# YannDubs/disentangling-vae

Hardware: NVIDIA H100
Metric: images/sec (higher is better)
Workload: dtype f32

## Files before the change

disentangling-vae_b200/csrc/dv_conv_img.cu:

```cuda
#include "dv_common.cuh"

namespace dv {
namespace img {

constexpr int kThreads = 256;
constexpr int kLoPitch = 36;

__device__ __forceinline__ void cp_async16(void* smem_dst, const void* gsrc, bool valid) {
  const uint32_t d = (uint32_t)__cvta_generic_to_shared(smem_dst);
  const int sz = valid ? 16 : 0;
  asm volatile("cp.async.cg.shared.global [%0], [%1], 16, %2;" ::"r"(d), "l"(gsrc), "r"(sz) : "memory");
}
__device__ __forceinline__ void cp_async4(void* smem_dst, const void* gsrc, bool valid) {
  const uint32_t d = (uint32_t)__cvta_generic_to_shared(smem_dst);
  const int sz = valid ? 4 : 0;
  asm volatile("cp.async.ca.shared.global [%0], [%1], 4, %2;" ::"r"(d), "l"(gsrc), "r"(sz) : "memory");
}
__device__ __forceinline__ void cp_async_wait_all() { asm volatile("cp.async.wait_all;" ::: "memory"); }

template <int CH, int W, int TR>
__device__ __forceinline__ void load_hi_tile(float* __restrict__ s_hi, const float* __restrict__ hi, int b, int i0, int H) {
  constexpr int IN_ROWS = 2 * TR + 2, COLS = 2 * W + 2, PITCH = 2 * W + 4;
  const int HH = 2 * H, WW = 2 * W;
#pragma unroll 4
  for (int e = threadIdx.x; e < CH * IN_ROWS * COLS; e += kThreads) {
    const int xx = e % COLS, rr = (e / COLS) % IN_ROWS, c = e / (COLS * IN_ROWS);
    const int iy = 2 * i0 - 1 + rr, ix = xx - 1;
    const bool ok = (unsigned)iy < (unsigned)HH && (unsigned)ix < (unsigned)WW;
    cp_async4(s_hi + (c * IN_ROWS + rr) * PITCH + xx, ok ? hi + ((long long)(b * CH + c) * HH + iy) * WW + ix : hi, ok);
  }
}

template <int CH, int W>
__global__ void __launch_bounds__(kThreads, 2)
img_down_kernel(const float* __restrict__ hi, const float* __restrict__ wd, const float* __restrict__ bias,
                const float* __restrict__ mask, float* __restrict__ lo, int B, int H, int act,
                float* __restrict__ colsum_part, const uint32_t* __restrict__ mask_bits, uint32_t* __restrict__ bits_out) {
  constexpr int TR = 16;
  constexpr int PXG = (TR * W) / 64;
  constexpr int CB = W / PXG;
  constexpr int NX = 2 * PXG + 2;
  constexpr int IN_ROWS = 2 * TR + 2, PITCH = 2 * W + 4;
  __shared__ __align__(16) float s_w[kTaps * CH * kLoCh];
  __shared__ __align__(16) float s_hi[CH * IN_ROWS * PITCH];
  __shared__ __align__(16) float s_bias[kLoCh];
  __shared__ float s_cs[kThreads / 32][kLoCh];
  const int tid = threadIdx.x, lane = tid & 31, warp = tid >> 5;
  for (int i = tid; i < kTaps * CH * kLoCh; i += kThreads) s_w[i] = wd[i];
  if (tid < kLoCh) s_bias[tid] = bias ? bias[tid] : 0.f;
  const int cg = tid & 3, pg = tid >> 2;
  const int r_thr = pg / CB, c0 = (pg % CB) * PXG;
  const int tiles_per_img = H / TR;
  const int num_tiles = B * tiles_per_img;
  float csum[8];
#pragma unroll
  for (int k = 0; k < 8; ++k) csum[k] = 0.f;
  for (int tile = blockIdx.x; tile < num_tiles; tile += gridDim.x) {
    const int b = tile / tiles_per_img, i0 = (tile % tiles_per_img) * TR;
    __syncthreads();
    load_hi_tile<CH, W, TR>(s_hi, hi, b, i0, H);
    const long long p0 = ((long long)b * H + i0 + r_thr) * W + c0;
    uint32_t mb_lo = 0xffffffffu, mb_hi = 0xffffffffu;
    if (mask_bits) {
      mb_lo = 0u; mb_hi = 0u;
#pragma unroll
      for (int i = 0; i < PXG; ++i) {
        const uint32_t mw = __ldg(mask_bits + p0 + i);
        mb_lo |= ((mw >> (4 * cg)) & 15u) << (4 * i);
        mb_hi |= ((mw >> (16 + 4 * cg)) & 15u) << (4 * i);
      }
    } else if (mask) {
      mb_lo = 0u; mb_hi = 0u;
#pragma unroll
      for (int i = 0; i < PXG; ++i) {
        const float* mk = mask + (p0 + i) * kLoCh + 4 * cg;
        const float4 a = ldg4(mk), d = ldg4(mk + 16);
        mb_lo |= ((a.x > 0.f ? 1u : 0u) | (a.y > 0.f ? 2u : 0u) | (a.z > 0.f ? 4u : 0u) | (a.w > 0.f ? 8u : 0u)) << (4 * i);
        mb_hi |= ((d.x > 0.f ? 1u : 0u) | (d.y > 0.f ? 2u : 0u) | (d.z > 0.f ? 4u : 0u) | (d.w > 0.f ? 8u : 0u)) << (4 * i);
      }
    }
    cp_async_wait_all();
    __syncthreads();
    float acc[PXG][8];
#pragma unroll
    for (int i = 0; i < PXG; ++i)
#pragma unroll
      for (int k = 0; k < 8; ++k) acc[i][k] = 0.f;
#pragma unroll
    for (int c = 0; c < CH; ++c) {
#pragma unroll
      for (int kh = 0; kh < 4; ++kh) {
        float x[NX];
        const float* row = s_hi + (c * IN_ROWS + 2 * r_thr + kh) * PITCH + 2 * c0;
#pragma unroll
        for (int v = 0; v < NX / 2; ++v) {
          const float2 t2 = *reinterpret_cast<const float2*>(row + 2 * v);
          x[2 * v] = t2.x; x[2 * v + 1] = t2.y;
        }
#pragma unroll
        for (int kw = 0; kw < 4; ++kw) {
          const float* wp = s_w + ((kh * 4 + kw) * CH + c) * kLoCh + 4 * cg;
          const float4 wa = *reinterpret_cast<const float4*>(wp), wb = *reinterpret_cast<const float4*>(wp + 16);
#pragma unroll
          for (int i = 0; i < PXG; ++i) {
            const float xv = x[2 * i + kw];
            acc[i][0] = fmaf(xv, wa.x, acc[i][0]); acc[i][1] = fmaf(xv, wa.y, acc[i][1]);
            acc[i][2] = fmaf(xv, wa.z, acc[i][2]); acc[i][3] = fmaf(xv, wa.w, acc[i][3]);
            acc[i][4] = fmaf(xv, wb.x, acc[i][4]); acc[i][5] = fmaf(xv, wb.y, acc[i][5]);
            acc[i][6] = fmaf(xv, wb.z, acc[i][6]); acc[i][7] = fmaf(xv, wb.w, acc[i][7]);
          }
        }
      }
    }
    const float4 ba = *reinterpret_cast<const float4*>(s_bias + 4 * cg), bb = *reinterpret_cast<const float4*>(s_bias + 16 + 4 * cg);
    const float bv[8] = {ba.x, ba.y, ba.z, ba.w, bb.x, bb.y, bb.z, bb.w};
#pragma unroll
    for (int i = 0; i < PXG; ++i) {
      float v[8];
#pragma unroll
      for (int k = 0; k < 8; ++k) {
        float t = acc[i][k] + bv[k];
        if (act == DV_ACT_RELU) t = fmaxf(t, 0.f);
        const uint32_t bit = ((k < 4 ? mb_lo : mb_hi) >> (4 * i + (k & 3))) & 1u;
        v[k] = bit ? t : 0.f;
        csum[k] += v[k];
      }
      float* dst = lo + (p0 + i) * kLoCh + 4 * cg;
      *reinterpret_cast<float4*>(dst) = make_float4(v[0], v[1], v[2], v[3]);
      *reinterpret_cast<float4*>(dst + 16) = make_float4(v[4], v[5], v[6], v[7]);
      if (bits_out) {
        uint32_t ob = 0u;
#pragma unroll
        for (int k = 0; k < 8; ++k) ob |= (v[k] > 0.f ? 1u : 0u) << ((k < 4 ? 0 : 16) + 4 * cg + (k & 3));
        ob |= __shfl_xor_sync(0xffffffffu, ob, 1);
        ob |= __shfl_xor_sync(0xffffffffu, ob, 2);
        if (cg == 0) bits_out[p0 + i] = ob;
      }
    }
  }
  if (colsum_part) {
#pragma unroll
    for (int k = 0; k < 8; ++k) {
      float t = csum[k];
      t += __shfl_xor_sync(0xffffffffu, t, 4); t += __shfl_xor_sync(0xffffffffu, t, 8); t += __shfl_xor_sync(0xffffffffu, t, 16);
      if (lane < 4) s_cs[warp][(k < 4 ? 0 : 16) + 4 * lane + (k & 3)] = t;
    }
    __syncthreads();
    if (warp == 0) {
      float t = 0.f;
#pragma unroll
      for (int w2 = 0; w2 < kThreads / 32; ++w2) t += s_cs[w2][lane];
      colsum_part[blockIdx.x * kLoCh + lane] = t;
    }
  }
}

template <int CH, int W>
__global__ void __launch_bounds__(kThreads, (CH == 1) ? 2 : 1)
img_wgrad_kernel(const float* __restrict__ lo, const float* __restrict__ hi, float* __restrict__ ws, int B, int H) {
  constexpr int TR = (W == 32) ? 16 : 16;
  constexpr int IN_ROWS = 2 * TR + 2, PITCH = 2 * W + 4;
  constexpr int NPX = TR * W;
  constexpr int NSTREAM = kThreads / 16;
  extern __shared__ __align__(16) float smem[];
  float* s_lo = smem;
  float* s_hi = smem + NPX * kLoPitch;
  const int tid = threadIdx.x;
  const int stream = tid >> 4, st = tid & 15;
  const int cl4 = st & 7, half = st >> 3;
  float acc[CH][8][4];
  float bsum[4] = {0.f, 0.f, 0.f, 0.f};
#pragma unroll
  for (int c = 0; c < CH; ++c)
#pragma unroll
    for (int t = 0; t < 8; ++t)
#pragma unroll
      for (int e = 0; e < 4; ++e) acc[c][t][e] = 0.f;
  const int tiles_per_img = H / TR;
  const int num_tiles = B * tiles_per_img;
  for (int tile = blockIdx.x; tile < num_tiles; tile += gridDim.x) {
    const int b = tile / tiles_per_img, i0 = (tile % tiles_per_img) * TR;
    __syncthreads();
    load_hi_tile<CH, W, TR>(s_hi, hi, b, i0, H);
    {
      const float4* src = reinterpret_cast<const float4*>(lo + ((long long)b * H + i0) * W * kLoCh);
#pragma unroll 4
      for (int e = tid; e < NPX * 8; e += kThreads) {
        const int px = e >> 3, j = e & 7;
        cp_async16(s_lo + px * kLoPitch + 4 * j, src + e, true);
      }
    }
    cp_async_wait_all();
    __syncthreads();
#pragma unroll 2
    for (int px = stream; px < NPX; px += NSTREAM) {
      const int r = px / W, cc = px % W;
      const float4 l4 = *reinterpret_cast<const float4*>(s_lo + px * kLoPitch + 4 * cl4);
      if (half == 0) { bsum[0] += l4.x; bsum[1] += l4.y; bsum[2] += l4.z; bsum[3] += l4.w; }
#pragma unroll
      for (int c = 0; c < CH; ++c) {
#pragma unroll
        for (int rr = 0; rr < 2; ++rr) {
          const float* row = s_hi + (c * IN_ROWS + 2 * r + 2 * half + rr) * PITCH + 2 * cc;
          const float2 a = *reinterpret_cast<const float2*>(row), d = *reinterpret_cast<const float2*>(row + 2);
          const float xv[4] = {a.x, a.y, d.x, d.y};
#pragma unroll
          for (int kw = 0; kw < 4; ++kw) {
            acc[c][rr * 4 + kw][0] = fmaf(xv[kw], l4.x, acc[c][rr * 4 + kw][0]);
            acc[c][rr * 4 + kw][1] = fmaf(xv[kw], l4.y, acc[c][rr * 4 + kw][1]);
            acc[c][rr * 4 + kw][2] = fmaf(xv[kw], l4.z, acc[c][rr * 4 + kw][2]);
            acc[c][rr * 4 + kw][3] = fmaf(xv[kw], l4.w, acc[c][rr * 4 + kw][3]);
          }
        }
      }
    }
  }
  __syncthreads();
  constexpr int K = kTaps * CH;
  float* red = smem;
  {
    float* mine = red + stream * (K + 1) * kLoCh;
#pragma unroll
    for (int c = 0; c < CH; ++c)
#pragma unroll
      for (int t = 0; t < 8; ++t) {
        const int tap = (2 * half + (t >> 2)) * 4 + (t & 3);
#pragma unroll
        for (int e = 0; e < 4; ++e) mine[(tap * CH + c) * kLoCh + 4 * cl4 + e] = acc[c][t][e];
      }
    if (half == 0) {
#pragma unroll
      for (int e = 0; e < 4; ++e) mine[K * kLoCh + 4 * cl4 + e] = bsum[e];
    }
  }
  __syncthreads();
  float* out = ws + (long long)blockIdx.x * (K + 1) * kLoCh;
  for (int idx = tid; idx < (K + 1) * kLoCh; idx += kThreads) {
    float s = 0.f;
#pragma unroll
    for (int q = 0; q < NSTREAM; ++q) s += red[q * (K + 1) * kLoCh + idx];
    out[idx] = s;
  }
}

template <int CH, int W>
__global__ void __launch_bounds__(128, 2)
img_up_kernel(const float* __restrict__ lo, const float* __restrict__ wu, const float* __restrict__ bias,
              float* __restrict__ hi, int B, int H, int act) {
  constexpr int NT = 128;
  constexpr int PY = 2;
  constexpr int TCOLS = W / 2;
  constexpr int TROWS = NT / TCOLS;
  constexpr int TR = TROWS * PY;
  constexpr int SW = W + 2;
  extern __shared__ __align__(16) float smem[];
  float* s_lo = smem;
  float* s_w = smem + (TR + 2) * SW * kLoCh;
  const int tid = threadIdx.x;
  for (int i = tid; i < kTaps * CH * kLoCh; i += NT) s_w[i] = wu[i];
  const int tn = tid % TCOLS, tm = tid / TCOLS;
  const int tiles_per_img = (H + TR - 1) / TR;
  const int num_tiles = B * tiles_per_img;
  const int HH = 2 * H, WW = 2 * W;
  for (int tile = blockIdx.x; tile < num_tiles; tile += gridDim.x) {
    const int b = tile / tiles_per_img, m0 = (tile % tiles_per_img) * TR;
    __syncthreads();
#pragma unroll 4
    for (int e = tid; e < (TR + 2) * SW * 8; e += NT) {
      const int j = e & 7, xx = (e >> 3) % SW, rr = (e >> 3) / SW;
      const int m = m0 - 1 + rr, n = xx - 1;
      const bool ok = (unsigned)m < (unsigned)H && (unsigned)n < (unsigned)W;
      cp_async16(s_lo + (rr * SW + xx) * kLoCh + 4 * (j ^ ((xx >> 1) & 7)),
                 ok ? lo + (((long long)b * H + m) * W + n) * kLoCh + 4 * j : lo, ok);
    }
    cp_async_wait_all();
    __syncthreads();
    if (m0 + PY * tm < H) {
      float out[CH][2 * PY][4];
#pragma unroll
      for (int c = 0; c < CH; ++c)
#pragma unroll
        for (int y = 0; y < 2 * PY; ++y)
#pragma unroll
          for (int x = 0; x < 4; ++x) out[c][y][x] = 0.f;
      const float* base = s_lo + ((PY * tm) * SW + 2 * tn) * kLoCh;
#pragma unroll 1
      for (int j = 0; j < 8; ++j) {
        float4 nb[PY + 2][4];
#pragma unroll
        for (int rr = 0; rr < PY + 2; ++rr)
#pragma unroll
          for (int xx = 0; xx < 4; ++xx)
            nb[rr][xx] = *reinterpret_cast<const float4*>(base + (rr * SW + xx) * kLoCh + 4 * (j ^ ((tn + (xx >> 1)) & 7)));
#pragma unroll
        for (int c = 0; c < CH; ++c) {
#pragma unroll
          for (int tap = 0; tap < kTaps; ++tap) {
            const int kh = tap >> 2, kw = tap & 3;
            const float4 w4 = *reinterpret_cast<const float4*>(s_w + (tap * CH + c) * kLoCh + 4 * j);
            const int py = (kh & 1) ? 0 : 1, dm = (kh == 1 || kh == 2) ? 0 : ((kh == 3) ? -1 : 1);
            const int px = (kw & 1) ? 0 : 1, dn = (kw == 1 || kw == 2) ? 0 : ((kw == 3) ? -1 : 1);
#pragma unroll
            for (int a = 0; a < PY; ++a)
#pragma unroll
              for (int d = 0; d < 2; ++d) {
                const float4 v = nb[a + 1 + dm][d + 1 + dn];
                float o = out[c][2 * a + py][2 * d + px];
                o = fmaf(v.x, w4.x, o); o = fmaf(v.y, w4.y, o); o = fmaf(v.z, w4.z, o); o = fmaf(v.w, w4.w, o);
                out[c][2 * a + py][2 * d + px] = o;
              }
          }
        }
      }
#pragma unroll
      for (int c = 0; c < CH; ++c) {
        const float bv = bias ? __ldg(bias + c) : 0.f;
#pragma unroll
        for (int y = 0; y < 2 * PY; ++y) {
          const int oy = 2 * (m0 + PY * tm) + y;
          if (oy < HH) {
            float v[4];
#pragma unroll
            for (int x = 0; x < 4; ++x) v[x] = apply_act(out[c][y][x] + bv, act, 0.f);
            *reinterpret_cast<float4*>(hi + ((long long)(b * CH + c) * HH + oy) * WW + 4 * tn) = make_float4(v[0], v[1], v[2], v[3]);
          }
        }
      }
    }
  }
}

template <int W> constexpr int up_tile_rows() { return (128 / (W / 2)) * 2; }
template <int CH, int W> constexpr size_t up_smem() {
  return (size_t)((up_tile_rows<W>() + 2) * (W + 2) * kLoCh + kTaps * CH * kLoCh) * sizeof(float);
}
template <int CH, int W> constexpr size_t wgrad_smem() {
  constexpr size_t tiles = (size_t)16 * W * kLoPitch + (size_t)CH * 34 * (2 * W + 4);
  constexpr size_t red = (size_t)(kThreads / 16) * (kTaps * CH + 1) * kLoCh;
  return (tiles > red ? tiles : red) * sizeof(float);
}

template <typename K>
static bool set_smem(K kernel, size_t bytes) {
  return bytes <= 48 * 1024 || cudaFuncSetAttribute(kernel, cudaFuncAttributeMaxDynamicSharedMemorySize, (int)bytes) == cudaSuccess;
}

int conv_down(const float* hi, const float* wd, const float* bias, const float* mask, const uint32_t* mask_bits, float* lo,
              uint32_t* bits_out, int B, int H, int W, int CH,
              int act, cudaStream_t st, float* colsum_part, int* nparts, int max_parts) {
  const int tiles = B * (H / 16);
  int grid = tiles < 2 * kNumSMs ? tiles : 2 * kNumSMs;
  if (colsum_part && grid > max_parts) grid = max_parts;
#define DV_IMG_DOWN(CHV, WV) \
  img_down_kernel<CHV, WV><<<grid, kThreads, 0, st>>>(hi, wd, bias, mask, lo, B, H, act, colsum_part, mask_bits, bits_out)
  if (CH == 1 && W == 32) DV_IMG_DOWN(1, 32);
  else if (CH == 3 && W == 32) DV_IMG_DOWN(3, 32);
  else if (CH == 1 && W == 16) DV_IMG_DOWN(1, 16);
  else DV_IMG_DOWN(3, 16);
#undef DV_IMG_DOWN
  *nparts = colsum_part ? grid : 0;
  return check_launch();
}

int wgrad_splits(int B, int H, int CH) {
  const int tiles = B * (H / 16);
  const int per_sm = (CH == 1) ? 2 : 1;
  return tiles < per_sm * kNumSMs ? tiles : per_sm * kNumSMs;
}

int conv_wgrad(const float* lo, const float* hi, float* ws, int B, int H, int W, int CH, cudaStream_t st) {
  const int grid = wgrad_splits(B, H, CH);
#define DV_IMG_WG(CHV, WV)                                                                     \
  do {                                                                                         \
    if (!set_smem(img_wgrad_kernel<CHV, WV>, wgrad_smem<CHV, WV>())) return DV_ERR_CUDA;       \
    img_wgrad_kernel<CHV, WV><<<grid, kThreads, wgrad_smem<CHV, WV>(), st>>>(lo, hi, ws, B, H); \
  } while (0)
  if (CH == 1 && W == 32) DV_IMG_WG(1, 32);
  else if (CH == 3 && W == 32) DV_IMG_WG(3, 32);
  else if (CH == 1 && W == 16) DV_IMG_WG(1, 16);
  else DV_IMG_WG(3, 16);
#undef DV_IMG_WG
  return check_launch();
}

int conv_up(const float* lo, const float* wu, const float* bias, float* hi, int B, int H, int W, int CH, int act, cudaStream_t st) {
#define DV_IMG_UP(CHV, WV)                                                                     \
  do {                                                                                         \
    const int tiles = B * ((H + up_tile_rows<WV>() - 1) / up_tile_rows<WV>());                \
    const int grid = tiles < 2 * kNumSMs ? tiles : 2 * kNumSMs;                                \
    if (!set_smem(img_up_kernel<CHV, WV>, up_smem<CHV, WV>())) return DV_ERR_CUDA;             \
    img_up_kernel<CHV, WV><<<grid, 128, up_smem<CHV, WV>(), st>>>(lo, wu, bias, hi, B, H, act); \
  } while (0)
  if (CH == 1 && W == 32) DV_IMG_UP(1, 32);
  else if (CH == 3 && W == 32) DV_IMG_UP(3, 32);
  else if (CH == 1 && W == 16) DV_IMG_UP(1, 16);
  else DV_IMG_UP(3, 16);
#undef DV_IMG_UP
  return check_launch();
}

}
}
```

disentangling-vae_b200/csrc/dv_ptx.cuh:

```cuda
#pragma once
#include <cuda.h>
#include <cuda_runtime.h>
#include <stdint.h>

namespace dv {
namespace ptx {

__device__ __forceinline__ uint32_t smem_u32(const void* p) {
  return static_cast<uint32_t>(__cvta_generic_to_shared(p));
}

__device__ __forceinline__ void mbar_init(uint64_t* bar, uint32_t count) {
  asm volatile("mbarrier.init.shared::cta.b64 [%0], %1;" ::"r"(smem_u32(bar)), "r"(count));
}
__device__ __forceinline__ void fence_mbar_init() {
  asm volatile("fence.mbarrier_init.release.cluster;" ::: "memory");
}
__device__ __forceinline__ void mbar_arrive(uint64_t* bar) {
  asm volatile("mbarrier.arrive.shared::cta.b64 _, [%0];" ::"r"(smem_u32(bar)) : "memory");
}
__device__ __forceinline__ void mbar_arrive_expect_tx(uint64_t* bar, uint32_t bytes) {
  asm volatile("mbarrier.arrive.expect_tx.shared::cta.b64 _, [%0], %1;" ::"r"(smem_u32(bar)), "r"(bytes) : "memory");
}
__device__ __forceinline__ void mbar_wait(uint64_t* bar, uint32_t parity) {
  const uint32_t addr = smem_u32(bar);
  uint32_t done = 0;
  for (uint32_t spin = 0; !done; ++spin) {
    asm volatile(
        "{\n\t.reg .pred p;\n\t"
        "mbarrier.try_wait.parity.shared::cta.b64 p, [%1], %2;\n\t"
        "selp.u32 %0, 1, 0, p;\n\t}"
        : "=r"(done)
        : "r"(addr), "r"(parity)
        : "memory");
    if (spin > (1u << 24)) __trap();
  }
}

__device__ __forceinline__ uint32_t lds32(uint32_t smem_addr) {
  uint32_t v;
  asm volatile("ld.shared.u32 %0, [%1];" : "=r"(v) : "r"(smem_addr) : "memory");
  return v;
}

__device__ __forceinline__ void sts128(uint32_t smem_addr, const uint32_t (&v)[4]) {
  asm volatile("st.shared.v4.u32 [%0], {%1, %2, %3, %4};" ::"r"(smem_addr), "r"(v[0]), "r"(v[1]), "r"(v[2]), "r"(v[3]) : "memory");
}
__device__ __forceinline__ void fence_proxy_async() { asm volatile("fence.proxy.async.shared::cta;" ::: "memory"); }

__device__ __forceinline__ uint32_t swz128(int r, int c) {
  return (uint32_t)(r * 128 + ((((c >> 2) ^ (r & 7)) << 4) | ((c & 3) << 2)));
}

__device__ __forceinline__ void prefetch_tmap(const CUtensorMap* m) {
  asm volatile("prefetch.tensormap [%0];" ::"l"(reinterpret_cast<uint64_t>(m)) : "memory");
}
__device__ __forceinline__ void tma_load_4d(void* smem_dst, const CUtensorMap* m, uint64_t* bar, int c0, int c1, int c2, int c3) {
  asm volatile(
      "cp.async.bulk.tensor.4d.shared::cluster.global.mbarrier::complete_tx::bytes [%0], [%1, {%3, %4, %5, %6}], [%2];"
      ::"r"(smem_u32(smem_dst)), "l"(reinterpret_cast<uint64_t>(m)), "r"(smem_u32(bar)), "r"(c0), "r"(c1), "r"(c2), "r"(c3)
      : "memory");
}
__device__ __forceinline__ void tma_load_2d(void* smem_dst, const CUtensorMap* m, uint64_t* bar, int c0, int c1) {
  asm volatile(
      "cp.async.bulk.tensor.2d.shared::cluster.global.mbarrier::complete_tx::bytes [%0], [%1, {%3, %4}], [%2];"
      ::"r"(smem_u32(smem_dst)), "l"(reinterpret_cast<uint64_t>(m)), "r"(smem_u32(bar)), "r"(c0), "r"(c1)
      : "memory");
}
__device__ __forceinline__ void tma_prefetch_4d(const CUtensorMap* m, int c0, int c1, int c2, int c3) {
  asm volatile("cp.async.bulk.prefetch.tensor.4d.L2.global.tile [%0, {%1, %2, %3, %4}];"
               ::"l"(reinterpret_cast<uint64_t>(m)), "r"(c0), "r"(c1), "r"(c2), "r"(c3) : "memory");
}

typedef CUresult (*EncodeTiledFn)(CUtensorMap*, CUtensorMapDataType, cuuint32_t, void*, const cuuint64_t*, const cuuint64_t*,
                                  const cuuint32_t*, const cuuint32_t*, CUtensorMapInterleave, CUtensorMapSwizzle,
                                  CUtensorMapL2promotion, CUtensorMapFloatOOBfill);
inline EncodeTiledFn get_encode() {
  static const EncodeTiledFn fn = [] {
    void* p = nullptr;
    cudaDriverEntryPointQueryResult qres;
    const bool ok = cudaGetDriverEntryPoint("cuTensorMapEncodeTiled", &p, cudaEnableDefault, &qres) == cudaSuccess &&
                    qres == cudaDriverEntryPointSuccess;
    return ok ? reinterpret_cast<EncodeTiledFn>(p) : nullptr;
  }();
  return fn;
}

__device__ __forceinline__ float tf32_round(float x) {
  return __uint_as_float((__float_as_uint(x) + 0x1000u) & 0xFFFFE000u);
}
__device__ __forceinline__ void split_tf32(uint32_t x, uint32_t& hi, uint32_t& lo) {
  const float h = tf32_round(__uint_as_float(x));
  hi = __float_as_uint(h);
  lo = __float_as_uint(tf32_round(__uint_as_float(x) - h));
}

__device__ __forceinline__ void mma_tf32(float (&d)[4], const uint32_t (&a)[4], const uint32_t (&b)[2]) {
  asm volatile(
      "mma.sync.aligned.m16n8k8.row.col.f32.tf32.tf32.f32 {%0, %1, %2, %3}, {%4, %5, %6, %7}, {%8, %9}, {%0, %1, %2, %3};"
      : "+f"(d[0]), "+f"(d[1]), "+f"(d[2]), "+f"(d[3])
      : "r"(a[0]), "r"(a[1]), "r"(a[2]), "r"(a[3]), "r"(b[0]), "r"(b[1]));
}

__device__ __forceinline__ void mma_3xtf32(float (&main)[4], float (&corr)[4], const uint32_t (&a_hi)[4],
                                           const uint32_t (&a_lo)[4], const uint32_t (&b_hi)[2], const uint32_t (&b_lo)[2]) {
  mma_tf32(main, a_hi, b_hi);
  mma_tf32(corr, a_hi, b_lo);
  mma_tf32(corr, a_lo, b_hi);
}

__device__ __forceinline__ uint64_t wgmma_desc_k128(uint32_t smem_addr) {
  return (uint64_t)((smem_addr & 0x3FFFFu) >> 4) | ((uint64_t)1 << 16) | ((uint64_t)(1024 >> 4) << 32) | ((uint64_t)1 << 62);
}
__device__ __forceinline__ void wgmma_fence() { asm volatile("wgmma.fence.sync.aligned;" ::: "memory"); }
__device__ __forceinline__ void wgmma_commit() { asm volatile("wgmma.commit_group.sync.aligned;" ::: "memory"); }
template <int N>
__device__ __forceinline__ void wgmma_wait() { asm volatile("wgmma.wait_group.sync.aligned %0;" ::"n"(N) : "memory"); }
template <int N>
__device__ __forceinline__ void fence_regs(float (&r)[N]) {
#pragma unroll
  for (int i = 0; i < N; ++i) asm volatile("" : "+f"(r[i])::"memory");
}

__device__ __forceinline__ void wgmma_m64n32k8_rs(float (&d)[16], const uint32_t* a, uint64_t b_desc, int accumulate) {
  asm volatile(
      "{\n\t.reg .pred p;\n\tsetp.ne.b32 p, %21, 0;\n\t"
      "wgmma.mma_async.sync.aligned.m64n32k8.f32.tf32.tf32 "
      "{%0, %1, %2, %3, %4, %5, %6, %7, %8, %9, %10, %11, %12, %13, %14, %15}, "
      "{%16, %17, %18, %19}, %20, p, 1, 1;\n\t}"
      : "+f"(d[0]), "+f"(d[1]), "+f"(d[2]), "+f"(d[3]), "+f"(d[4]), "+f"(d[5]), "+f"(d[6]), "+f"(d[7]),
        "+f"(d[8]), "+f"(d[9]), "+f"(d[10]), "+f"(d[11]), "+f"(d[12]), "+f"(d[13]), "+f"(d[14]), "+f"(d[15])
      : "r"(a[0]), "r"(a[1]), "r"(a[2]), "r"(a[3]), "l"(b_desc), "r"(accumulate));
}

}
}
```

Baseline: 461,700.

## Double-buffer image conv tiles with cp.async and TMA bulk loads

Moves img_down_kernel to dynamic shared memory with a two-stage ring so the next hi tile is prefetched via cp.async while the current tile is computed. img_wgrad_kernel splits each 16-row tile into two 8-row units, double-buffers them, and loads the lo activations with a single bulk async copy tracked by an mbarrier instead of per-thread 16-byte cp.async. The aim is to hide global load latency behind compute. In exchange it uses more shared memory in the down kernel, which may lower occupancy, and drops the padded lo pitch, which could add shared-memory bank conflicts.

```diff
diff --git a/disentangling-vae_b200/csrc/dv_conv_img.cu b/disentangling-vae_b200/csrc/dv_conv_img.cu
--- a/disentangling-vae_b200/csrc/dv_conv_img.cu
+++ b/disentangling-vae_b200/csrc/dv_conv_img.cu
@@ -1,22 +1,29 @@
 #include "dv_common.cuh"
+#include "dv_ptx.cuh"
 
 namespace dv {
 namespace img {
 
+using namespace ptx;
+
 constexpr int kThreads = 256;
-constexpr int kLoPitch = 36;
-
+constexpr int kStages = 2;
+
+__device__ __forceinline__ void cp_async4(void* smem_dst, const void* gsrc, bool valid) {
+  const uint32_t d = (uint32_t)__cvta_generic_to_shared(smem_dst);
+  const int sz = valid ? 4 : 0;
+  asm volatile("cp.async.ca.shared.global [%0], [%1], 4, %2;" ::"r"(d), "l"(gsrc), "r"(sz) : "memory");
+}
 __device__ __forceinline__ void cp_async16(void* smem_dst, const void* gsrc, bool valid) {
   const uint32_t d = (uint32_t)__cvta_generic_to_shared(smem_dst);
   const int sz = valid ? 16 : 0;
   asm volatile("cp.async.cg.shared.global [%0], [%1], 16, %2;" ::"r"(d), "l"(gsrc), "r"(sz) : "memory");
 }
-__device__ __forceinline__ void cp_async4(void* smem_dst, const void* gsrc, bool valid) {
-  const uint32_t d = (uint32_t)__cvta_generic_to_shared(smem_dst);
-  const int sz = valid ? 4 : 0;
-  asm volatile("cp.async.ca.shared.global [%0], [%1], 4, %2;" ::"r"(d), "l"(gsrc), "r"(sz) : "memory");
-}
 __device__ __forceinline__ void cp_async_wait_all() { asm volatile("cp.async.wait_all;" ::: "memory"); }
+__device__ __forceinline__ void cp_async_commit() { asm volatile("cp.async.commit_group;" ::: "memory"); }
+__device__ __forceinline__ void cp_async_wait_stage() {
+  asm volatile("cp.async.wait_group %0;" ::"n"(kStages - 1) : "memory");
+}
 
 template <int CH, int W, int TR>
 __device__ __forceinline__ void load_hi_tile(float* __restrict__ s_hi, const float* __restrict__ hi, int b, int i0, int H) {
@@ -30,21 +37,30 @@
     cp_async4(s_hi + (c * IN_ROWS + rr) * PITCH + xx, ok ? hi + ((long long)(b * CH + c) * HH + iy) * WW + ix : hi, ok);
   }
 }
+template <int CH, int W, int TR> __host__ __device__ constexpr int hi_tile_floats() { return CH * (2 * TR + 2) * (2 * W + 4); }
+
+constexpr int kDownTR = 16;
+template <int CH, int W> __host__ __device__ constexpr size_t down_smem() {
+  return (size_t)(kTaps * CH * kLoCh + kLoCh + (kThreads / 32) * kLoCh + kStages * hi_tile_floats<CH, W, kDownTR>()) *
+         sizeof(float);
+}
 
 template <int CH, int W>
 __global__ void __launch_bounds__(kThreads, 2)
 img_down_kernel(const float* __restrict__ hi, const float* __restrict__ wd, const float* __restrict__ bias,
                 const float* __restrict__ mask, float* __restrict__ lo, int B, int H, int act,
                 float* __restrict__ colsum_part, const uint32_t* __restrict__ mask_bits, uint32_t* __restrict__ bits_out) {
-  constexpr int TR = 16;
+  constexpr int TR = kDownTR;
   constexpr int PXG = (TR * W) / 64;
   constexpr int CB = W / PXG;
   constexpr int NX = 2 * PXG + 2;
   constexpr int IN_ROWS = 2 * TR + 2, PITCH = 2 * W + 4;
-  __shared__ __align__(16) float s_w[kTaps * CH * kLoCh];
-  __shared__ __align__(16) float s_hi[CH * IN_ROWS * PITCH];
-  __shared__ __align__(16) float s_bias[kLoCh];
-  __shared__ float s_cs[kThreads / 32][kLoCh];
+  constexpr int HI_TILE = hi_tile_floats<CH, W, TR>();
+  extern __shared__ __align__(16) float smem[];
+  float* s_w = smem;
+  float* s_bias = s_w + kTaps * CH * kLoCh;
+  float* s_cs = s_bias + kLoCh;
+  float* s_hi = s_cs + (kThreads / 32) * kLoCh;
   const int tid = threadIdx.x, lane = tid & 31, warp = tid >> 5;
   for (int i = tid; i < kTaps * CH * kLoCh; i += kThreads) s_w[i] = wd[i];
   if (tid < kLoCh) s_bias[tid] = bias ? bias[tid] : 0.f;
@@ -52,13 +68,26 @@
   const int r_thr = pg / CB, c0 = (pg % CB) * PXG;
   const int tiles_per_img = H / TR;
   const int num_tiles = B * tiles_per_img;
+#pragma unroll
+  for (int s = 0; s < kStages - 1; ++s) {
+    const int t = blockIdx.x + s * gridDim.x;
+    if (t < num_tiles) load_hi_tile<CH, W, TR>(s_hi + s * HI_TILE, hi, t / tiles_per_img, (t % tiles_per_img) * TR, H);
+    cp_async_commit();
+  }
   float csum[8];
 #pragma unroll
   for (int k = 0; k < 8; ++k) csum[k] = 0.f;
-  for (int tile = blockIdx.x; tile < num_tiles; tile += gridDim.x) {
+  int n = 0;
+  for (int tile = blockIdx.x; tile < num_tiles; tile += gridDim.x, ++n) {
     const int b = tile / tiles_per_img, i0 = (tile % tiles_per_img) * TR;
     __syncthreads();
-    load_hi_tile<CH, W, TR>(s_hi, hi, b, i0, H);
+    {
+      const int t = tile + (kStages - 1) * gridDim.x;
+      if (t < num_tiles)
+        load_hi_tile<CH, W, TR>(s_hi + ((n + kStages - 1) % kStages) * HI_TILE, hi, t / tiles_per_img, (t % tiles_per_img) * TR, H);
+      cp_async_commit();
+    }
+    const float* s_t = s_hi + (n % kStages) * HI_TILE;
     const long long p0 = ((long long)b * H + i0 + r_thr) * W + c0;
     uint32_t mb_lo = 0xffffffffu, mb_hi = 0xffffffffu;
     if (mask_bits) {
@@ -79,7 +108,7 @@
         mb_hi |= ((d.x > 0.f ? 1u : 0u) | (d.y > 0.f ? 2u : 0u) | (d.z > 0.f ? 4u : 0u) | (d.w > 0.f ? 8u : 0u)) << (4 * i);
       }
     }
-    cp_async_wait_all();
+    cp_async_wait_stage();
     __syncthreads();
     float acc[PXG][8];
 #pragma unroll
@@ -91,7 +120,7 @@
 #pragma unroll
       for (int kh = 0; kh < 4; ++kh) {
         float x[NX];
-        const float* row = s_hi + (c * IN_ROWS + 2 * r_thr + kh) * PITCH + 2 * c0;
+        const float* row = s_t + (c * IN_ROWS + 2 * r_thr + kh) * PITCH + 2 * c0;
 #pragma unroll
         for (int v = 0; v < NX / 2; ++v) {
           const float2 t2 = *reinterpret_cast<const float2*>(row + 2 * v);
@@ -143,31 +172,61 @@
     for (int k = 0; k < 8; ++k) {
       float t = csum[k];
       t += __shfl_xor_sync(0xffffffffu, t, 4); t += __shfl_xor_sync(0xffffffffu, t, 8); t += __shfl_xor_sync(0xffffffffu, t, 16);
-      if (lane < 4) s_cs[warp][(k < 4 ? 0 : 16) + 4 * lane + (k & 3)] = t;
+      if (lane < 4) s_cs[warp * kLoCh + (k < 4 ? 0 : 16) + 4 * lane + (k & 3)] = t;
     }
     __syncthreads();
     if (warp == 0) {
       float t = 0.f;
 #pragma unroll
-      for (int w2 = 0; w2 < kThreads / 32; ++w2) t += s_cs[w2][lane];
+      for (int w2 = 0; w2 < kThreads / 32; ++w2) t += s_cs[w2 * kLoCh + lane];
       colsum_part[blockIdx.x * kLoCh + lane] = t;
     }
   }
+}
+
+constexpr int kWgTR = 16;
+constexpr int kWgSR = 8;
+template <int W> __host__ __device__ constexpr int wg_lo_floats() { return kWgSR * W * kLoCh; }
+template <int CH, int W> __host__ __device__ constexpr int wg_stage_floats() { return wg_lo_floats<W>() + hi_tile_floats<CH, W, kWgSR>(); }
+template <int CH, int W> __host__ __device__ constexpr size_t wgrad_smem() {
+  constexpr size_t ring = (size_t)kStages * wg_stage_floats<CH, W>();
+  constexpr size_t red = (size_t)(kThreads / 16) * (kTaps * CH + 1) * kLoCh;
+  return (ring > red ? ring : red) * sizeof(float) + 16 * kStages;
 }
 
 template <int CH, int W>
 __global__ void __launch_bounds__(kThreads, (CH == 1) ? 2 : 1)
 img_wgrad_kernel(const float* __restrict__ lo, const float* __restrict__ hi, float* __restrict__ ws, int B, int H) {
-  constexpr int TR = (W == 32) ? 16 : 16;
-  constexpr int IN_ROWS = 2 * TR + 2, PITCH = 2 * W + 4;
-  constexpr int NPX = TR * W;
+  constexpr int IN_ROWS = 2 * kWgSR + 2, PITCH = 2 * W + 4;
+  constexpr int NPX = kWgSR * W;
   constexpr int NSTREAM = kThreads / 16;
+  constexpr int STAGE = wg_stage_floats<CH, W>();
+  constexpr uint32_t LO_BYTES = wg_lo_floats<W>() * sizeof(float);
+  constexpr size_t RING_FLOATS = (wgrad_smem<CH, W>() - 16 * kStages) / sizeof(float);
   extern __shared__ __align__(16) float smem[];
-  float* s_lo = smem;
-  float* s_hi = smem + NPX * kLoPitch;
+  uint64_t* full = reinterpret_cast<uint64_t*>(smem + RING_FLOATS);
   const int tid = threadIdx.x;
   const int stream = tid >> 4, st = tid & 15;
   const int cl4 = st & 7, half = st >> 3;
+  const int tiles_per_img = H / kWgTR;
+  const int num_tiles = B * tiles_per_img;
+  const int my_tiles = blockIdx.x < num_tiles ? (num_tiles - 1 - blockIdx.x) / gridDim.x + 1 : 0;
+  const int units = 2 * my_tiles;
+  auto issue = [&](int u) {
+    float* stage = smem + (u % kStages) * STAGE;
+    const int tile = blockIdx.x + (u >> 1) * gridDim.x;
+    const int b = tile / tiles_per_img, i0 = (tile % tiles_per_img) * kWgTR + (u & 1) * kWgSR;
+    if (tid == 0) {
+      mbar_arrive_expect_tx(&full[u % kStages], LO_BYTES);
+      bulk_load(stage, lo + ((long long)b * H + i0) * W * kLoCh, LO_BYTES, &full[u % kStages]);
+    }
+    load_hi_tile<CH, W, kWgSR>(stage + wg_lo_floats<W>(), hi, b, i0, H);
+  };
+  if (tid == 0) {
+    for (int s = 0; s < kStages; ++s) mbar_init(&full[s], 1);
+    fence_mbar_init();
+  }
+  __syncthreads();
   float acc[CH][8][4];
   float bsum[4] = {0.f, 0.f, 0.f, 0.f};
 #pragma unroll
@@ -176,26 +235,23 @@
     for (int t = 0; t < 8; ++t)
 #pragma unroll
       for (int e = 0; e < 4; ++e) acc[c][t][e] = 0.f;
-  const int tiles_per_img = H / TR;
-  const int num_tiles = B * tiles_per_img;
-  for (int tile = blockIdx.x; tile < num_tiles; tile += gridDim.x) {
-    const int b = tile / tiles_per_img, i0 = (tile % tiles_per_img) * TR;
-    __syncthreads();
-    load_hi_tile<CH, W, TR>(s_hi, hi, b, i0, H);
-    {
-      const float4* src = reinterpret_cast<const float4*>(lo + ((long long)b * H + i0) * W * kLoCh);
-#pragma unroll 4
-      for (int e = tid; e < NPX * 8; e += kThreads) {
-        const int px = e >> 3, j = e & 7;
-        cp_async16(s_lo + px * kLoPitch + 4 * j, src + e, true);
-      }
-    }
-    cp_async_wait_all();
-    __syncthreads();
+#pragma unroll
+  for (int s = 0; s < kStages - 1; ++s) {
+    if (s < units) issue(s);
+    cp_async_commit();
+  }
+  for (int u = 0; u < units; ++u) {
+    if (u + kStages - 1 < units) issue(u + kStages - 1);
+    cp_async_commit();
+    cp_async_wait_stage();
+    mbar_wait(&full[u % kStages], (u / kStages) & 1);
+    __syncthreads();
+    const float* s_lo = smem + (u % kStages) * STAGE;
+    const float* s_hi = s_lo + wg_lo_floats<W>();
 #pragma unroll 2
     for (int px = stream; px < NPX; px += NSTREAM) {
       const int r = px / W, cc = px % W;
-      const float4 l4 = *reinterpret_cast<const float4*>(s_lo + px * kLoPitch + 4 * cl4);
+      const float4 l4 = *reinterpret_cast<const float4*>(s_lo + px * kLoCh + 4 * cl4);
       if (half == 0) { bsum[0] += l4.x; bsum[1] += l4.y; bsum[2] += l4.z; bsum[3] += l4.w; }
 #pragma unroll
       for (int c = 0; c < CH; ++c) {
@@ -214,8 +270,8 @@
         }
       }
     }
-  }
-  __syncthreads();
+    __syncthreads();
+  }
   constexpr int K = kTaps * CH;
   float* red = smem;
   {
@@ -330,14 +386,9 @@
   }
 }
 
-template <int W> constexpr int up_tile_rows() { return (128 / (W / 2)) * 2; }
-template <int CH, int W> constexpr size_t up_smem() {
+template <int W> __host__ __device__ constexpr int up_tile_rows() { return (128 / (W / 2)) * 2; }
+template <int CH, int W> __host__ __device__ constexpr size_t up_smem() {
   return (size_t)((up_tile_rows<W>() + 2) * (W + 2) * kLoCh + kTaps * CH * kLoCh) * sizeof(float);
-}
-template <int CH, int W> constexpr size_t wgrad_smem() {
-  constexpr size_t tiles = (size_t)16 * W * kLoPitch + (size_t)CH * 34 * (2 * W + 4);
-  constexpr size_t red = (size_t)(kThreads / 16) * (kTaps * CH + 1) * kLoCh;
-  return (tiles > red ? tiles : red) * sizeof(float);
 }
 
 template <typename K>
@@ -348,11 +399,15 @@
 int conv_down(const float* hi, const float* wd, const float* bias, const float* mask, const uint32_t* mask_bits, float* lo,
               uint32_t* bits_out, int B, int H, int W, int CH,
               int act, cudaStream_t st, float* colsum_part, int* nparts, int max_parts) {
-  const int tiles = B * (H / 16);
+  const int tiles = B * (H / kDownTR);
   int grid = tiles < 2 * kNumSMs ? tiles : 2 * kNumSMs;
   if (colsum_part && grid > max_parts) grid = max_parts;
-#define DV_IMG_DOWN(CHV, WV) \
-  img_down_kernel<CHV, WV><<<grid, kThreads, 0, st>>>(hi, wd, bias, mask, lo, B, H, act, colsum_part, mask_bits, bits_out)
+#define DV_IMG_DOWN(CHV, WV)                                                                                   \
+  do {                                                                                                         \
+    if (!set_smem(img_down_kernel<CHV, WV>, down_smem<CHV, WV>())) return DV_ERR_CUDA;                         \
+    img_down_kernel<CHV, WV><<<grid, kThreads, down_smem<CHV, WV>(), st>>>(hi, wd, bias, mask, lo, B, H, act,  \
+                                                                             colsum_part, mask_bits, bits_out); \
+  } while (0)
   if (CH == 1 && W == 32) DV_IMG_DOWN(1, 32);
   else if (CH == 3 && W == 32) DV_IMG_DOWN(3, 32);
   else if (CH == 1 && W == 16) DV_IMG_DOWN(1, 16);
@@ -363,7 +418,7 @@
 }
 
 int wgrad_splits(int B, int H, int CH) {
-  const int tiles = B * (H / 16);
+  const int tiles = B * (H / kWgTR);
   const int per_sm = (CH == 1) ? 2 : 1;
   return tiles < per_sm * kNumSMs ? tiles : per_sm * kNumSMs;
 }
diff --git a/disentangling-vae_b200/csrc/dv_ptx.cuh b/disentangling-vae_b200/csrc/dv_ptx.cuh
--- a/disentangling-vae_b200/csrc/dv_ptx.cuh
+++ b/disentangling-vae_b200/csrc/dv_ptx.cuh
@@ -67,6 +67,11 @@
       ::"r"(smem_u32(smem_dst)), "l"(reinterpret_cast<uint64_t>(m)), "r"(smem_u32(bar)), "r"(c0), "r"(c1)
       : "memory");
 }
+__device__ __forceinline__ void bulk_load(void* smem_dst, const void* gsrc, uint32_t bytes, uint64_t* bar) {
+  asm volatile("cp.async.bulk.shared::cluster.global.mbarrier::complete_tx::bytes [%0], [%1], %2, [%3];"
+               ::"r"(smem_u32(smem_dst)), "l"(reinterpret_cast<uint64_t>(gsrc)), "r"(bytes), "r"(smem_u32(bar))
+               : "memory");
+}
 __device__ __forceinline__ void tma_prefetch_4d(const CUtensorMap* m, int c0, int c1, int c2, int c3) {
   asm volatile("cp.async.bulk.prefetch.tensor.4d.L2.global.tile [%0, {%1, %2, %3, %4}];"
                ::"l"(reinterpret_cast<uint64_t>(m)), "r"(c0), "r"(c1), "r"(c2), "r"(c3) : "memory");
```

Result: no change. 466,700, median of 6 (+1.1%).
